# tan9zj/xnrs

Hardware: AMD Instinct MI355X
Metric: impressions/sec (encode+score) on MIND-shaped batches (higher is better)
Workload: dtype f32; 1 GPU; NRMS full user+news encode + 5-candidate dot scoring (BASELINE configs[2]; token shape of config/mind_small_NRMS.yml); batch_impressions_per_gpu=512, history=50, candidates=5, d_backbone=768, n_heads=16, emb_dim=256, parallelism=impressions sharded by user over 1 GPU(s), no data-path collective

## Files before the change

### include/xnrs_hip.h

```cpp
#ifndef XNRS_HIP_H
#define XNRS_HIP_H

#include <stddef.h>
#include <stdint.h>

#ifdef __cplusplus
extern "C" {
#endif

#define XNRS_ABI_VERSION 6

#define XNRS_OK 0
#define XNRS_EINVAL (-1)
#define XNRS_EHEADS (-2)
#define XNRS_EWORKSPACE (-3)
#define XNRS_EUNSUPPORTED (-4)

#define XNRS_ACT_NONE 0
#define XNRS_ACT_RELU 1
#define XNRS_ACT_TANH 2

#define XNRS_POOL_ADDITIVE 0
#define XNRS_POOL_MEAN 1

// ... 210 lines not shown

#define XNRS_PROFILE_STAGES 10
int32_t xnrs_profile_enable(uint32_t stage_mask);
int32_t xnrs_profile_read(double *ms, int64_t *launches, double *flops);

int32_t xnrs_qkv_launch_count(int32_t reset);
int32_t xnrs_qkv_one_launch_map(int64_t block, int64_t live_tiles, int64_t live_rows, int32_t kv_row_tiles,
                                int32_t kv_col_tiles, int64_t q_rows, int32_t q_tile_rows, int32_t q_col_tiles,
                                int32_t *section, int32_t *index);

int32_t xnrs_fc1_in_tail_count(int32_t reset);
int32_t xnrs_qkv_fc1_launch_map(int64_t block, int64_t live_tiles, int64_t live_rows, int64_t fc1_live_rows,
                                int32_t kv_row_tiles, int32_t kv_col_tiles, int64_t q_rows, int32_t q_tile_rows,
                                int32_t q_col_tiles, int64_t fc1_rows, int32_t fc1_tile_rows, int32_t fc1_col_tiles,
                                int32_t *section, int32_t *index);

int32_t xnrs_train_fold_enabled(void);

#define XNRS_STATUS_NONBINARY_MASK 1
#define XNRS_STATUS_ROW_RANGE 2
#define XNRS_STATUS_QUERY_RANGE 4
int32_t xnrs_set_status_word(int32_t *device_word);
const char *xnrs_status_string(int32_t word);

#define XNRS_GEMM_F32 0
#define XNRS_GEMM_BF16X3 1
#define XNRS_GEMM_BF16X2 2
int32_t xnrs_set_gemm_mode(int32_t mode);
int32_t xnrs_get_gemm_mode(void);

// ... 136 lines not shown
```

### xnrs_amd/csrc/api.hip

```cpp
#include <mutex>
#include <vector>

#include "host.h"

using namespace xnrs;

namespace xnrs {
uint32_t g_prof_mask = 0;
}
namespace {
std::vector<ProfRec> g_prof;
std::mutex g_prof_mu;
constexpr size_t PROF_MAX = 1 << 16;
}

bool xnrs::prof_begin(ProfRec* r, hipStream_t stream) {
  if (hipEventCreate(&r->beg) != hipSuccess || hipEventCreate(&r->end) != hipSuccess) return false;
  (void)hipEventRecord(r->beg, stream);
  return true;
}

void xnrs::prof_end(const ProfRec& r, hipStream_t stream) {
  (void)hipEventRecord(r.end, stream);
  std::lock_guard<std::mutex> lk(g_prof_mu);
// ... 79 lines not shown
  if (grid > 0x7fffffffLL) return XNRS_EINVAL;
  if (section && index) {
    const xnrs::QkvOneLaunchWork w =
        xnrs::qkv_one_launch_map(block, live_tiles, live_rows, kv_row_tiles, kv_col_tiles, q_rows, q_tile_rows, q_col_tiles);
    *section = w.section;
    *index = w.index;
  }
  return (int32_t)grid;
}

int32_t xnrs_fc1_in_tail_count(int32_t reset) {
  const int64_t n = xnrs::fc1_in_tail_read(reset != 0);
  return n > 0x7fffffffLL ? 0x7fffffff : (int32_t)n;
}

int32_t xnrs_qkv_fc1_launch_map(int64_t block, int64_t live_tiles, int64_t live_rows, int64_t fc1_live_rows, int32_t kv_row_tiles,
                                int32_t kv_col_tiles, int64_t q_rows, int32_t q_tile_rows, int32_t q_col_tiles, int64_t fc1_rows,
                                int32_t fc1_tile_rows, int32_t fc1_col_tiles, int32_t* section, int32_t* index) {
  if (kv_row_tiles < 0 || kv_col_tiles < 1 || q_rows < 0 || q_tile_rows < 1 || q_col_tiles < 1 || fc1_rows < 0 || fc1_tile_rows < 1 ||
      fc1_col_tiles < 1)
    return XNRS_EINVAL;
  const int64_t grid =
      xnrs::qkv_fc1_launch_grid(kv_row_tiles, kv_col_tiles, q_rows, q_tile_rows, q_col_tiles, fc1_rows, fc1_tile_rows, fc1_col_tiles);
  if (grid > 0x7fffffffLL) return XNRS_EINVAL;
  if (section && index) {
    const xnrs::QkvOneLaunchWork w = xnrs::qkv_fc1_launch_map(block, live_tiles, live_rows, fc1_live_rows, kv_row_tiles, kv_col_tiles, q_rows,
                                                              q_tile_rows, q_col_tiles, fc1_rows, fc1_tile_rows, fc1_col_tiles);
    *section = w.section;
    *index = w.index;
  }
// ... 42 lines not shown
```

### xnrs_amd/csrc/batch.hip

```cpp
#include <atomic>

#include "host.h"

namespace xnrs {

__device__ __forceinline__ uint64_t mix64(uint64_t seed, uint64_t a, uint64_t b) {
  uint64_t z = seed + 0x9E3779B97F4A7C15ull * (a * 0x100000001B3ull + b + 1);
  z = (z ^ (z >> 30)) * 0xBF58476D1CE4E5B9ull;
  z = (z ^ (z >> 27)) * 0x94D049BB133111EBull;
  return z ^ (z >> 31);
}

__global__ __launch_bounds__(256) void assemble_train_kernel(BatchArgs a) {
  const int64_t i = (int64_t)blockIdx.x * 256 + threadIdx.x;
  const int W = a.l_hist + 1 + a.n_neg;
  if (i >= a.B * W) return;
  const int64_t b = i / W;
  const int j = (int)(i - b * W);
  const int64_t s = a.sess[b];
  if (j < a.l_hist) {
    const int64_t lo = a.hist_off[s], hi = a.hist_off[s + 1];
    const int64_t n = (hi - lo < a.l_hist) ? (hi - lo) : a.l_hist;
    a.hist_out[b * a.l_hist + j] = (j < n) ? a.hist_val[hi - n + j] : a.pad_row;
  } else {
// ... 395 lines not shown
        w += __popcll(b);
        if (kept && sl < S) kv_src[e1 + sl] = (int32_t)(src0 + sl);
      }
      if (lane == 0) kv_block[j] = e1 / S;
    }
    __syncthreads();
  }
  bad = __syncthreads_or(bad);
  if (tid == 0) {
    counts[0] = s_carry[0];
    counts[1] = s_carry[1];
    counts[2] = bad ? 1 : 0;
  }
}

struct DenseLists {
  int32_t* live_loc;
  uint8_t* alive;
  int64_t* n_tiles;
  int32_t* tiles;
  int64_t cap;
  int BM;
};
__device__ void list_live_tiles(const uint8_t* __restrict__ alive, int64_t cn, int L, int BM, int32_t* __restrict__ tiles,
                                int64_t* __restrict__ n_out, int* s_wsum, int* s_carry);

template <bool DENSE>
__global__ __launch_bounds__(1024) void compact_rows64_kernel(const float* __restrict__ mask, const int32_t* __restrict__ ids,
                                                               int64_t n_news, int64_t chunk, int S, int64_t* __restrict__ row_off_all,
                                                               int32_t* __restrict__ live_all, int32_t* __restrict__ kvs_all,
                                                               int32_t* __restrict__ kvb_all, int64_t* __restrict__ counts_all,
                                                               DenseLists dl) {
  __shared__ unsigned long long s_bits[1024];
  __shared__ int64_t s_row[1024];
  __shared__ int s_ex[2][1024];
  __shared__ int s_wsum[2][16];
  __shared__ int s_carry[2];
  const int tid = threadIdx.x, wave = tid >> 6, lane = tid & 63;
  const int64_t news0 = (int64_t)blockIdx.x * chunk;
  const int cn = (int)(n_news - news0 < chunk ? n_news - news0 : chunk);
  int64_t* row_off = DENSE ? nullptr : row_off_all + (int64_t)blockIdx.x * (chunk + 1);
  int32_t* live_src = live_all ? live_all + (int64_t)blockIdx.x * chunk * S : nullptr;
  int32_t* kv_src = DENSE ? nullptr : kvs_all + (int64_t)blockIdx.x * chunk * S;
  int32_t* kv_block = DENSE ? nullptr : kvb_all + (int64_t)blockIdx.x * chunk;
  int64_t* counts = counts_all + 3 * (int64_t)blockIdx.x;
  int32_t* live_loc = DENSE ? dl.live_loc + (int64_t)blockIdx.x * chunk * S : nullptr;
  uint8_t* alive = DENSE ? dl.alive + news0 : nullptr;
  int bad = 0;
  if (tid < 2) s_carry[tid] = 0;
  if (!DENSE && tid == 0) row_off[0] = 0;
  for (int base = 0; base < cn; base += 1024) {
    const int nn = cn - base < 1024 ? cn - base : 1024;
    s_bits[tid] = 0ull;
    s_row[tid] = tid < nn ? (ids ? (int64_t)ids[news0 + base + tid] : news0 + base + tid) : 0;
    __syncthreads();
    const int n_el = nn * S;
    for (int i0 = tid; i0 < n_el; i0 += 4096) {
      float mv[4];
      int jj[4], sl[4];
#pragma unroll
      for (int u = 0; u < 4; ++u) {
        const int i = i0 + 1024 * u;
        jj[u] = (i < n_el ? i : 0) / S;
        sl[u] = (i < n_el ? i : 0) - jj[u] * S;
        mv[u] = i < n_el ? mask[s_row[jj[u]] * S + sl[u]] : 0.f;
// ... 13 lines not shown
      int x = v[which];
      for (int off = 1; off < 64; off <<= 1) {
        const int up = __shfl_up(x, off);
        if (lane >= off) x += up;
      }
      incl[which] = x;
      if (lane == 63) s_wsum[which][wave] = x;
    }
    __syncthreads();
    for (int which = 0; which < 2; ++which) {
      int before = s_carry[which];
      for (int w = 0; w < wave; ++w) before += s_wsum[which][w];
      s_ex[which][tid] = before + incl[which] - v[which];
    }
    if (tid < nn) {
      if constexpr (DENSE) {
        alive[base + tid] = bits != 0ull ? 1 : 0;
      } else {
        row_off[base + tid + 1] = s_ex[0][tid] + cnt;
        kv_block[base + tid] = s_ex[1][tid] / S;
      }
    }
    __syncthreads();
    if (tid == 1023) {
      s_carry[0] = s_ex[0][1023] + v[0];
      s_carry[1] = s_ex[1][1023] + v[1];
    }
#pragma unroll 4
    for (int i = tid; i < n_el; i += 1024) {
      const int jj = i / S, sl = i - jj * S;
      const unsigned long long b = s_bits[jj];
      if (b == 0ull) continue;
      const int32_t src = (int32_t)(s_row[jj] * S + sl);
      if constexpr (DENSE) {
        if ((b >> sl) & 1ull) {
          const int at = s_ex[0][jj] + __popcll(b & ((1ull << sl) - 1ull));
          live_loc[at] = (int32_t)((base + jj) * S + sl);
          if (live_src) live_src[at] = src;
        }
      } else {
        kv_src[s_ex[1][jj] + sl] = src;
        if ((b >> sl) & 1ull) live_src[s_ex[0][jj] + __popcll(b & ((1ull << sl) - 1ull))] = src;
      }
    }
    __syncthreads();
  }
  if constexpr (DENSE) {
    if (tid == 0) {
      counts[0] = s_carry[0];
      counts[1] = s_carry[1];
      s_carry[0] = 0;
    }
    __syncthreads();
    list_live_tiles(alive, cn, S, dl.BM, dl.tiles + (int64_t)blockIdx.x * dl.cap, dl.n_tiles + blockIdx.x, s_wsum[0], &s_carry[0]);
    return;
  }
  bad = __syncthreads_or(bad);
  if (tid == 0) {
    counts[0] = s_carry[0];
    counts[1] = s_carry[1];
    counts[2] = bad ? 1 : 0;
  }
}

__global__ __launch_bounds__(256) void row_counts_kernel(const float* __restrict__ mask, const int32_t* __restrict__ ids,
                                                          int64_t n_seq, int L, int32_t* __restrict__ cnt) {
  const int lane = threadIdx.x & 63;
  const int64_t seq = (int64_t)blockIdx.x * 4 + (threadIdx.x >> 6);
  if (seq >= n_seq) return;
  const float* mp = mask + (ids ? (int64_t)ids[seq] : seq) * L;
// ... 126 lines not shown
  return w;
}
void set_status_word(int32_t* w) {
  int dev = -1;
  (void)hipGetDevice(&dev);
  g_status_device.store(w ? dev : -1, std::memory_order_relaxed);
  g_status_word.store(w, std::memory_order_relaxed);
}

hipError_t launch_compact_rows(const float* mask, const int32_t* ids, int64_t n_news, int64_t chunk, int S, int64_t* row_off,
                               int32_t* live_src, int32_t* kv_src, int32_t* kv_block, int64_t* counts, hipStream_t stream) {
  if (n_news <= 0 || chunk <= 0) return hipSuccess;
  const int64_t passes = (n_news + chunk - 1) / chunk;
  if (passes > 0x7fffffffLL) return hipErrorInvalidValue;
  if (S <= 64)
    hipLaunchKernelGGL(compact_rows64_kernel<false>, dim3((unsigned)passes), dim3(1024), 0, stream, mask, ids, n_news, chunk, S,
                       row_off, live_src, kv_src, kv_block, counts, DenseLists{});
  else
    hipLaunchKernelGGL(compact_rows_kernel, dim3((unsigned)passes), dim3(1024), 0, stream, mask, ids, n_news, chunk, S, row_off,
                       live_src, kv_src, kv_block, counts);
  return hipGetLastError();
}

__global__ __launch_bounds__(1024) void live_tiles_kernel(const float* __restrict__ mask, const int32_t* __restrict__ ids,
                                                           int64_t n_seq, int64_t chunk, int L, int BM, int64_t cap,
                                                           uint8_t* __restrict__ alive_all, int64_t* __restrict__ n_tiles,
                                                           int32_t* __restrict__ tiles_all) {
  __shared__ int s_wsum[16];
  __shared__ int s_carry;
  const int tid = threadIdx.x;
  const int64_t seq0 = (int64_t)blockIdx.x * chunk;
  const int64_t cn = n_seq - seq0 < chunk ? n_seq - seq0 : chunk;
  uint8_t* alive = alive_all + seq0;
  int32_t* tiles = tiles_all + (int64_t)blockIdx.x * cap;
  for (int64_t j = tid; j < cn; j += 1024) {
    const float* mp = mask + (ids ? (int64_t)ids[seq0 + j] : seq0 + j) * L;
    int any = 0;
// ... 35 lines not shown
  }
  if (tid == 0) *n_out = *s_carry;
}

hipError_t launch_live_tiles(const float* mask, const int32_t* ids, int64_t n_seq, int64_t chunk, int L, int BM, uint8_t* alive,
                             int64_t* n_tiles, int32_t* tiles, hipStream_t stream) {
  if (n_seq <= 0 || chunk <= 0 || L <= 0 || BM <= 0) return hipSuccess;
  const int64_t passes = (n_seq + chunk - 1) / chunk;
  const int64_t cap = live_tiles_cap(chunk, L, BM);
  if (passes > 0x7fffffffLL || cap > 0x7fffffffLL) return hipErrorInvalidValue;
  hipLaunchKernelGGL(live_tiles_kernel, dim3((unsigned)passes), dim3(1024), 0, stream, mask, ids, n_seq, chunk, L, BM, cap, alive,
                     n_tiles, tiles);
  return hipGetLastError();
}

hipError_t launch_dense_row_lists(const float* mask, const int32_t* ids, int64_t n_seq, int64_t chunk, int L, int BM,
                                  int32_t* live_loc, int32_t* live_src, int64_t* counts, uint8_t* alive, int64_t* n_tiles,
                                  int32_t* tiles, hipStream_t stream) {
  if (n_seq <= 0 || chunk <= 0 || L <= 0 || BM <= 0) return hipSuccess;
  const int64_t passes = (n_seq + chunk - 1) / chunk;
  const int64_t cap = live_tiles_cap(chunk, L, BM);
  if (L > 64 || passes > 0x7fffffffLL || cap > 0x7fffffffLL || chunk * L > 0x7fffffffLL) return hipErrorInvalidValue;
  hipLaunchKernelGGL(compact_rows64_kernel<true>, dim3((unsigned)passes), dim3(1024), 0, stream, mask, ids, n_seq, chunk, L,
                     nullptr, ids ? live_src : nullptr, nullptr, nullptr, counts, DenseLists{live_loc, alive, n_tiles, tiles, cap, BM});
  return hipGetLastError();
}

}

using namespace xnrs;

extern "C" {

size_t xnrs_row_lists_workspace_bytes(int64_t n_seq) { return n_seq > 0 ? align_up((size_t)n_seq * sizeof(int32_t)) : 0; }

int32_t xnrs_build_row_lists(const float* m, const int32_t* ids, int64_t n_seq, int32_t L, int32_t* live_rows,
                             int32_t* live_src_rows, int32_t* kv_rows, int32_t* kv_src_rows, int64_t* counts, void* ws,
                             size_t ws_bytes, void* stream) {
  if (n_seq < 0 || L <= 0 || !m || !live_rows || !kv_rows || !counts) return XNRS_EINVAL;
// ... 92 lines not shown
```

### xnrs_amd/csrc/encoder_fwd.hip

```cpp
#include <vector>

#include "host.h"

using namespace xnrs;

namespace xnrs {

Plan make_plan(int64_t n_seq, int L, int D, int A, int E, bool att, bool additive, bool head, bool pooled, int64_t chunk,
               bool train, int n_heads, bool widen) {
  Plan p{};
  if (train) chunk = n_seq > 0 ? n_seq : 1;
  if (chunk <= 0) chunk = 65536 / L;
  if (chunk > n_seq) chunk = n_seq;
  if (chunk < 1) chunk = 1;
  p.chunk = chunk;
  const size_t rows = (size_t)chunk * L;
  Carver c;
  p.off_qkv = c.take_if(att, rows * 3 * (size_t)D * F32);
  p.off_o = c.take_if(att, rows * (size_t)D * F32);
  p.off_y = c.take_if(att && pooled, rows * (size_t)D * F32);
  p.off_t = c.take_if(pooled && additive, rows * (size_t)A * F32);
  p.off_p = c.take_if(pooled && head, (size_t)n_seq * D * F32);
  p.off_h = c.take_if(pooled && head, (size_t)n_seq * E * F32);
  p.off_stats = c.take_if(train && att, (size_t)chunk * n_heads * L * 2 * F32);
// ... 210 lines not shown
    if (is_additive(r) && (!r.pool || !r.pool->w1 || !r.pool->w2 || r.pool->hidden <= 0)) return XNRS_EINVAL;
    if (r.pool_kind == XNRS_POOL_MEAN && !r.m) return XNRS_EINVAL;
    if (r.L > 512) return XNRS_EUNSUPPORTED;
    if (r.head && (!r.head->w0 || !r.head->w2 || r.head->out_features <= 0 || r.head->activation < 0 || r.head->activation > 2))
      return XNRS_EINVAL;
  }
  return (r.ids && !r.m && r.pooled && r.pool_kind == XNRS_POOL_MEAN) ? XNRS_EINVAL : XNRS_OK;
}

struct Route {
  bool fused, afused;
  bool qkv_given, live, kvl, lr_qkv, tail, lt_qkv, direct, a16;
  bool fold;
  bool lr_fc1, lt_fc1, rowdot;
  bool skip_dead, read_counts;
};

bool news_fused_route(const SeqEncode& r, const Plan& p, int A, bool fold, NewsFusedArgs* f) {
  const xnrs_mha_params* att = r.att;
  const int L = r.L, D = r.D;
  if (!(att && is_additive(r) && !r.train && !r.a_out && att->dropout_p == 0.f && gemm_mode() == 0 && knobs().news_fused &&
        news_fused_plan(L, D, att->n_heads, A, nullptr) && (D / att->n_heads) * att->n_heads == D &&
        (knobs().news_fused == 2 || (L >= 26 && r.n_seq >= 192))))
    return false;
  f->x = r.x; f->ids = r.ids; f->mask = r.m;
  f->wq = att->wq; f->bq = att->bq; f->wk = att->wk; f->bk = att->bk; f->wv = att->wv; f->bv = att->bv;
  f->wo = att->wo; f->bo = att->bo;
  f->w1 = r.pool->w1; f->b1 = r.pool->b1; f->w2 = r.pool->w2; f->b2 = r.pool->b2;
  f->img = at(r.ws, p.off_nf);
  f->p = pooled_dst(fold, at(r.ws, p.fold.po), r.head, at(r.ws, p.off_p), r.y);
// ... 49 lines not shown
                  device_counts_ok(xal, D, A, r.att, additive ? r.pool : nullptr);
  MhaCoreArgs probe{};
  if (lt && knobs().mha_skip_masked) {
    probe = mha_core_args(at(r.ws, p.off_qkv) + D, 3 * (int64_t)D, r.att, at(r.ws, p.off_o), p.chunk, L, D);
    probe.q = at(r.ws, p.off_qkv); probe.mask = r.m; probe.skip_dead = 1;
  }
  rt.lt_qkv = probe.skip_dead && mha_core_skips_dead(probe);
  rt.lt_fc1 = lt && additive && rt.rowdot;
  const bool lr = lt && knobs().gemm_live_rows && p.off_lr_cnt != 0 && L <= 64 && n_rows <= 0x7fffffffLL &&
                  n_rows >= knobs().gemm_live_rows_min_rows;
  rt.lr_qkv = lr && rt.lt_qkv && !rt.direct;
  rt.lr_fc1 = lr && rt.lt_fc1;
  rt.tail = rt.lr_qkv && rt.lr_fc1 && rt.fold && r.pooled && !r.ids && !r.x16 && knobs().gemm_fc1_in_tail && !prof_on(3);
  rt.read_counts = (rt.lt_qkv && prof_on(0)) || (rt.lt_fc1 && prof_on(3));
  rt.skip_dead = rt.live || (r.pooled && r.m && knobs().mha_skip_masked);
  return rt;
}

struct Call {
  const SeqEncode& r;
  hipStream_t stream;
  const Plan p;
  const Route rt;
  NewsFusedArgs nf; AdditiveFusedArgs af;
  const int L = r.L, D = r.D, A = hidden_of(r);
  const xnrs_mha_params* att = r.att;
  const xnrs_row_lists rl = r.rl ? *r.rl : xnrs_row_lists{};
  const int32_t *lvx = rt.live ? (r.ids ? rl.live_src_rows : rl.live_rows) : nullptr, *kvx = rt.kvl ? (r.ids ? rl.kv_src_rows : rl.kv_rows) : nullptr;
  const int64_t* cnt = rl.counts_dev;
  const int64_t n_live = cnt ? r.n_seq * L : rl.n_live, n_kv = cnt ? r.n_seq * L : rl.n_kv;
// ... 167 lines not shown
int32_t project(const Call& c, const Pass& pass, DeferredFc1* prev) {
  if (c.rt.qkv_given) return XNRS_OK;
  if (c.rt.live) return project_train_lists(c, pass);
  if (c.rt.lr_qkv) return project_live_rows(c, pass, prev);
  GemmArgs g = qkv_projection(pass.cx, {pass.xids, c.L}, c.att, 0, c.qkv, 3 * (int64_t)c.D, pass.rows, c.D, c.pqkv);
  if (c.rt.lt_qkv) over_live_tiles(&g, pass.ltn, pass.ltl);
  ProfScope ps(0, 2.0 * (c.rt.lt_qkv ? pass.lt_rows : (double)pass.rows) * 3.0 * c.D * c.D, c.stream);
  return hip_rc(c.rt.direct ? launch_gemm_a16(g, c.r.x16, c.stream) : launch_gemm_f32(g, c.stream));
}

int32_t attend(const Call& c, const Pass& pass) {
  MhaCoreArgs ma = mha_core_args(c.qkv + c.D, 3 * (int64_t)c.D, c.att, c.o, pass.nc, c.L, c.D);
  ma.q = c.qkv; ma.mask = pass.cm; ma.mask_gather_ids = pass.cids; ma.dropout_p = c.att->dropout_p;
  ma.seed = c.att->seed + (uint64_t)pass.c0 * (uint64_t)c.att->n_heads * 0x9E3779B97F4A7C15ull;
  ma.seed_dev = c.att->seed_dev; ma.stats = c.stats; ma.skip_dead = c.rt.skip_dead ? 1 : 0;
  if (c.rt.lt_qkv && !mha_core_skips_dead(ma)) return XNRS_EUNSUPPORTED;
  ProfScope ps(1, 4.0 * pass.rows * (double)c.L * c.D, c.stream);
  return hip_rc(launch_mha_core(ma, c.stream));
}

int32_t out_project_train_lists(const Call& c, const Pass& pass, float* dst) {
  const int D = c.D;
  ProfScope ps(2, 2.0 * (double)prof_count(2, c.cnt, 0, c.n_live, c.stream) * (double)D * D, c.stream);
  XNRS_TRY(hipMemsetAsync(dst, 0, (size_t)pass.rows * D * sizeof(float), c.stream));
  if (c.n_live <= 0) return XNRS_OK;
  GemmArgs og = gemm_linear(c.o, {}, D, c.att->wo, c.att->bo, dst, D, 0, D, D, XNRS_ACT_NONE, c.po);
  over_row_list(&og, c.rl.live_rows, nullptr, c.n_live, c.cnt, 0.4f);
  return hip_rc(launch_gemm_f32(og, c.stream));
}
int32_t out_project(const Call& c, Pass* pass) {
  float* dst = c.rt.fold ? c.o : (c.r.pooled ? c.yb : c.r.y + pass->c0 * (int64_t)c.L * c.D);
  pass->seq = dst; pass->seq_ids = nullptr;
  if (c.rt.fold) return XNRS_OK;
// ... 459 lines not shown
```

### xnrs_amd/csrc/gemm_f32.hip

```cpp
#include <atomic>
#include <cstdlib>
#include <type_traits>

#include "kernels.h"

namespace xnrs {

constexpr int KALIGN = 32;

__device__ __attribute__((aligned(16))) float g_zero_line[4] = {0.f, 0.f, 0.f, 0.f};

typedef unsigned u32x4 __attribute__((ext_vector_type(4)));
constexpr unsigned BUF_OOB = 0x40000000u;

template <int TM, int TN, bool A_COL, bool B_KN, bool VEC, int PIPE, int BK, bool BUF = false, int MINW = 2, bool GATH = false,
          int KG = 2, bool RDOT = false, bool MDEV = false, bool LIVE = false>
__global__ __launch_bounds__(256, MINW) void gemm_f32_kernel(const GemmArgs a, int m_tiles, int n_tiles_seg, int gn) {
#define XNRS_GEMM_BID blockIdx.x
#define XNRS_GEMM_NWG gridDim.x
#define XNRS_GEMM_LDS_TILES(A, B)                            \
  __shared__ __attribute__((aligned(16))) float A[NBUF][A_SZ]; \
  __shared__ __attribute__((aligned(16))) float B[NBUF][B_SZ];
#include "gemm_f32_body.h"
#undef XNRS_GEMM_BID
// ... 323 lines not shown
  k.mha_lds = (int)num("XNRS_MHA_LDS", -1);
  k.mha_headwave = num("XNRS_MHA_HEADWAVE", 1) != 0;
  k.mha_pair = num("XNRS_MHA_PAIR", 1) != 0;
  k.mha_bwd_fused = num("XNRS_MHA_BWD_FUSED", 1) != 0;
  k.gemm_dw = (int)num("XNRS_GEMM_DW", 2);
  k.gemm_dw_tile = (int)num("XNRS_GEMM_DW_TILE", 256);
  k.fold_out = (int)num("XNRS_FOLD_OUT", 1);
  k.fc1_rowdot = num("XNRS_FC1_ROWDOT", 1) != 0;
  k.fold_train = (int)num("XNRS_FOLD_TRAIN", 1);
  k.news_fused = (int)num("XNRS_NEWS_FUSED", 1);
  k.news_fused_npw = (int)num("XNRS_NEWS_FUSED_NPW", 0);
  k.fast_tanh = num("XNRS_FAST_TANH", 1) != 0;
  k.additive_fused = (int)num("XNRS_ADDITIVE_FUSED", 1);
  k.af_fbuf = num("XNRS_AF_FBUF", 1) == 2 ? 2 : 1;
  k.mha_skip_masked = num("XNRS_MHA_SKIP_MASKED", 1) != 0;
  {
    k.gemm_qkv_one_launch = num("XNRS_GEMM_QKV_ONE_LAUNCH", 1) != 0;
  }
  k.gemm_fc1_in_tail = num("XNRS_GEMM_FC1_IN_TAIL", 1) != 0;
  k.gemm_live_tiles = num("XNRS_GEMM_LIVE_TILES", 1) != 0;
  k.gemm_live_tiles_min_rows = num("XNRS_GEMM_LIVE_TILES_MIN_ROWS", 16384);
  k.gemm_live_rows = num("XNRS_GEMM_LIVE_ROWS", 1) != 0;
  k.gemm_live_rows_min_rows = num("XNRS_GEMM_LIVE_ROWS_MIN_ROWS", 16384);
  k.bwd_side_stream = num("XNRS_BWD_SIDE_STREAM", 1) != 0;
  k.bwd_side_min_rows = num("XNRS_BWD_SIDE_MIN_ROWS", 0);
  k.gru_layout = num("XNRS_GRU_LAYOUT", 0) == 1 ? 1 : 0;
  k.gemm_a16 = num("XNRS_GEMM_A16", 1) != 0;
  const long long m = num("XNRS_GEMM_MODE", 0);
  k.gemm_mode_init = (m >= 0 && m <= 2) ? (int)m : 0;
  return k;
// ... 157 lines not shown
```

### xnrs_amd/csrc/kernels.h

```cpp
#pragma once
#include <hip/hip_runtime.h>
#include <stdint.h>

namespace xnrs {

typedef float f32x4 __attribute__((ext_vector_type(4)));
typedef float f32x16 __attribute__((ext_vector_type(16)));
inline bool aligned16(const void* p) { return (reinterpret_cast<uintptr_t>(p) & 15) == 0; }

struct Knobs {
  int gemm_pipe = 6;
  int gemm_bk = 32;
  int gemm_buf = 1;
  long long gemm_group = -1;
  int gemm_tile = -1;
  long long split_min_tiles = 512;
  bool fc1_rowdot = true;
  int fold_train = 1;
  int fold_out = 1;
  int gemm_dw = 2;
  int gemm_dw_tile = 256;
  int mha_lds = -1;
  bool mha_pair = true;
  int mha_headwave = 1;
// ... 1 lines not shown
  int news_fused = 1;
  int news_fused_npw = 0;
  int gemm_mode_init = 0;
  bool fast_tanh = true;
  int additive_fused = 1;
  int af_fbuf = 1;
  bool bwd_side_stream = true;
  long long bwd_side_min_rows = 0;
  bool gemm_live_tiles = true;
  long long gemm_live_tiles_min_rows = 16384;
  bool gemm_live_rows = true;
  long long gemm_live_rows_min_rows = 16384;
  bool gemm_qkv_one_launch = true;
  bool gemm_fc1_in_tail = true;
  bool mha_skip_masked = true;
  bool gemm_a16 = true;
  int gru_layout = 0;
};
const Knobs& knobs();
void reload_knobs();

__device__ __forceinline__ int64_t load_dev_scalar(const int64_t* p) { return *p; }

struct GemmArgs {
  const float* A;
  int32_t a_col;
  const int32_t* gather_ids;
  int32_t gather_S;
  int32_t c_scatter;
  const int32_t* c_scatter_ids;
// ... 110 lines not shown
  const float* mask;
  const int32_t* mask_gather_ids;
  float* out;
  int64_t ldo;
  int64_t n_seq;
  int32_t S, n_heads, d_k;
  int32_t scaled;
  float dropout_p;
  uint64_t seed;
  const uint64_t* seed_dev;
  float* stats;
  const int64_t* q_off;
  int64_t ldq;
  const int32_t* kv_block;
  int32_t skip_dead;
};
hipError_t launch_mha_core(const MhaCoreArgs& a, hipStream_t stream);
bool mha_core_skips_dead(const MhaCoreArgs& a);

struct MhaBwdArgs {
  const float* q;
  const float* k;
  const float* v;
  int64_t ld;
  const float* mask;
  const int32_t* mask_gather_ids;
  const float* o;
  int64_t ldo;
  const float* d_o;
  int64_t lddo;
  const float* stats;
  float* delta;
  float* dq;
// ... 332 lines not shown
```

### xnrs_amd/csrc/mha_core.hip

```cpp
#include <cstdlib>

#include "kernels.h"

namespace xnrs {

template <int KT, bool VEC>
__global__ __launch_bounds__(256) void mha_core_kernel(MhaCoreArgs a, int QT, int64_t n_units) {
  const int lane = threadIdx.x & 63;
  const int64_t unit = (int64_t)blockIdx.x * 4 + (threadIdx.x >> 6);
  if (unit >= n_units) return;
  const int qt = (int)(unit % QT);
  const int64_t uh = unit / QT;
  const int hd = (int)(uh % a.n_heads);
  const int64_t seq = uh / a.n_heads;

  const int c = lane & 15, g = lane >> 4;
  const int S = a.S, dk = a.d_k;
  const int64_t row0 = seq * S;
  const int hoff = hd * dk;
  const int query = qt * 16 + c;
  const bool qvalid = query < S;

  f32x4 acc[KT];
#pragma unroll
// ... 423 lines not shown
  const float* vbase = a.v + kvbase;
  const int rem = TAIL ? S - KTM * 16 : 0;

  const int64_t q0 = a.q_off ? a.q_off[seq] : (int64_t)seq * S;
  const int nq = a.q_off ? (int)(a.q_off[seq + 1] - q0) : S;
  const int QT = (nq + 15) >> 4;
  if (nq == 0) return;
  const int c = lane & 15, g = lane >> 4;
  const int query = qt * 16 + c;
  const bool qvalid = query < nq;
  float mq = 1.f;
  if (a.mask && !a.q_off && qvalid) {
    const int64_t mrow = a.mask_gather_ids ? (int64_t)a.mask_gather_ids[seq] * S : (int64_t)seq * S;
    mq = a.mask[mrow + query];
  }
  if (a.skip_dead && a.mask && !a.q_off) {
    if (!__syncthreads_or(qvalid && mq != 0.f)) {
      if (qvalid) {
        float* orow = a.out + (q0 + query) * a.ldo + hd * dk;
#pragma unroll
        for (int dt = 0; dt < NFB; ++dt) {
          const int dv0 = dt * 16 + 4 * g;
          if (dv0 < dk) *reinterpret_cast<f32x4*>(orow + dv0) = f32x4{0.f, 0.f, 0.f, 0.f};
        }
        if (a.stats && g == 0) {
          float* sp = a.stats + (((int64_t)seq * a.n_heads + hd) * (int64_t)S + query) * 2;
          sp[0] = -1e9f;
          sp[1] = (float)S;
        }
      }
      return;
    }
  }
  const bool tile_dead = a.skip_dead && a.mask && !a.q_off && !__any(qvalid && mq != 0.f);
  const float* qrow = a.q_off ? a.q + (q0 + (qvalid ? query : 0)) * a.ldq + hd * dk
                              : a.q + hbase + (int64_t)(qvalid ? query : 0) * ld;
  f32x4 qf[NFB];
#pragma unroll
// ... 45 lines not shown
        }
      } else if (TAIL) {
#pragma unroll
        for (int r = 0; r < 4; ++r) Vt[r * NCH + vch] = vv[r];
      }
    }
  }
  __syncthreads();
  if (qt >= QT) return;
  if (tile_dead) {
    if (qvalid) {
      float* orow0 = a.out + (q0 + query) * a.ldo + hd * dk;
#pragma unroll
      for (int dt = 0; dt < NFB; ++dt) {
        const int dv0 = dt * 16 + 4 * g;
        if (dv0 < dk) *reinterpret_cast<f32x4*>(orow0 + dv0) = f32x4{0.f, 0.f, 0.f, 0.f};
      }
      if (a.stats && g == 0) {
        float* sp = a.stats + (((int64_t)seq * a.n_heads + hd) * (int64_t)S + query) * 2;
        sp[0] = -1e9f;
        sp[1] = (float)S;
      }
    }
    return;
  }

  f32x4 acc[KTM];
#pragma unroll
  for (int kt = 0; kt < KTM; ++kt) acc[kt] = f32x4{0.f, 0.f, 0.f, 0.f};
#pragma unroll
  for (int fb = 0; fb < NFB; ++fb) {
// ... 104 lines not shown
  if constexpr (TAIL) {
#pragma unroll
    for (int t = 0; t < 4; ++t) {
      if (t < rem) {
#pragma unroll
        for (int dt = 0; dt < NFB; ++dt) {
          const f32x4 vr = Vt[t * NCH + dt * 4 + g];
#pragma unroll
          for (int r = 0; r < 4; ++r) o[dt][r] = fmaf(st[t], vr[r], o[dt][r]);
        }
      }
    }
  }
  const int hoff = hd * dk;
  float* orow = a.out + (q0 + query) * a.ldo + hoff;
#pragma unroll
  for (int dt = 0; dt < NFB; ++dt) {
    const int dv0 = dt * 16 + 4 * g;
    if (qvalid && dv0 < dk) *reinterpret_cast<f32x4*>(orow + dv0) = o[dt];
  }
}

template <int KTM, int NFB, bool TAIL>
static hipError_t launch_pair_nfb(const MhaCoreArgs& a, hipStream_t stream) {
  const int64_t n_pairs = a.n_seq * a.n_heads;
  if (n_pairs > 0x7fffffffLL) return hipErrorInvalidValue;
  if (a.dropout_p > 0.f)
    hipLaunchKernelGGL((mha_core_pair_kernel<KTM, NFB, TAIL, true>), dim3((unsigned)n_pairs), dim3(256), 0, stream, a);
  else
    hipLaunchKernelGGL((mha_core_pair_kernel<KTM, NFB, TAIL, false>), dim3((unsigned)n_pairs), dim3(256), 0, stream, a);
  return hipGetLastError();
}

template <int KTM, bool TAIL>
// ... 42 lines not shown
  p.KT = (a.S + 15) / 16;
  p.fast = p.vec && a.S <= 64 && a.d_k <= 64 && ((int64_t)a.S * a.ld < (1ll << 31)) && knobs().mha_headwave;
  p.use_lds = a.q_off ? true : (knobs().mha_lds >= 0 ? knobs().mha_lds != 0 : (p.KT >= 3));
  const int rem = a.S & 15;
  p.tail = a.S > 16 && rem >= 1 && rem <= 4;
  p.KTM = p.tail ? a.S >> 4 : p.KT;
  p.pair = p.fast && p.use_lds && knobs().mha_pair && (int64_t)a.n_seq * a.S < (1ll << 31) &&
           (p.tail ? (p.KTM == 2 || p.KTM == 3) : (p.KTM == 3 || p.KTM == 4));
  return p;
}

bool mha_core_skips_dead(const MhaCoreArgs& a) {
  return a.skip_dead && a.mask && !a.q_off && a.S <= 128 && mha_pick(a).pair;
}

hipError_t launch_mha_core(const MhaCoreArgs& a, hipStream_t stream) {
  if (a.n_seq <= 0 || a.S <= 0) return hipSuccess;
  if (a.S > 128) return hipErrorInvalidValue;
  const MhaPick pk = mha_pick(a);
  const bool vec = pk.vec, fast = pk.fast, use_lds = pk.use_lds;
  const int KT = pk.KT;
  if (a.q_off && (!fast || a.stats || a.dropout_p > 0.f || a.ldq % 4 != 0)) return hipErrorInvalidValue;
  if (pk.pair) {
    const bool tail = pk.tail;
    const int KTM = pk.KTM;
    if (tail && KTM == 2) return launch_pair<2, true>(a, stream);
    if (tail && KTM == 3) return launch_pair<3, true>(a, stream);
    if (!tail && KTM == 3) return launch_pair<3, false>(a, stream);
    if (!tail && KTM == 4) return launch_pair<4, false>(a, stream);
  }
  if (fast && use_lds) {
    switch (KT) {
      case 1: return launch_lds_kt<1, 1>(a, stream);
      case 2: return launch_lds_kt<2, 2>(a, stream);
      case 3: return launch_lds_kt<3, 4>(a, stream);
      default: return launch_lds_kt<4, 4>(a, stream);
    }
// ... 23 lines not shown
```

Before: 21500 impressions/s.

## Skip attention output stores for masked rows and parallelize dense row lists

Adds an o_live_only mode to the pair MHA kernel. When a downstream fused path only reads live rows, it skips writing outputs for masked queries and dead sequences, which cuts global stores. It also replaces the single-block-per-pass dense row-list compaction with a new kernel that splits each pass into 64-row slices across many blocks. Each slice recomputes its prefix counts by rescanning earlier rows, so work is spread out at the cost of redundant mask reads. Masked output rows are now left uninitialized, which is only safe if every consumer reads live rows only.

```diff
diff --git a/include/xnrs_hip.h b/include/xnrs_hip.h
--- a/include/xnrs_hip.h
+++ b/include/xnrs_hip.h
@@ -248,6 +248,8 @@
                                 int32_t kv_row_tiles, int32_t kv_col_tiles, int64_t q_rows, int32_t q_tile_rows,
                                 int32_t q_col_tiles, int64_t fc1_rows, int32_t fc1_tile_rows, int32_t fc1_col_tiles,
                                 int32_t *section, int32_t *index);
+
+int32_t xnrs_mha_live_o_count(int32_t reset);
 
 int32_t xnrs_train_fold_enabled(void);
 
diff --git a/xnrs_amd/csrc/api.hip b/xnrs_amd/csrc/api.hip
--- a/xnrs_amd/csrc/api.hip
+++ b/xnrs_amd/csrc/api.hip
@@ -117,6 +117,11 @@
   return n > 0x7fffffffLL ? 0x7fffffff : (int32_t)n;
 }
 
+int32_t xnrs_mha_live_o_count(int32_t reset) {
+  const int64_t n = xnrs::mha_live_o_read(reset != 0);
+  return n > 0x7fffffffLL ? 0x7fffffff : (int32_t)n;
+}
+
 int32_t xnrs_qkv_fc1_launch_map(int64_t block, int64_t live_tiles, int64_t live_rows, int64_t fc1_live_rows, int32_t kv_row_tiles,
                                 int32_t kv_col_tiles, int64_t q_rows, int32_t q_tile_rows, int32_t q_col_tiles, int64_t fc1_rows,
                                 int32_t fc1_tile_rows, int32_t fc1_col_tiles, int32_t* section, int32_t* index) {
diff --git a/xnrs_amd/csrc/batch.hip b/xnrs_amd/csrc/batch.hip
--- a/xnrs_amd/csrc/batch.hip
+++ b/xnrs_amd/csrc/batch.hip
@@ -1,4 +1,5 @@
 #include <atomic>
+#include <type_traits>
 
 #include "host.h"
 
@@ -433,23 +434,10 @@
   }
 }
 
-struct DenseLists {
-  int32_t* live_loc;
-  uint8_t* alive;
-  int64_t* n_tiles;
-  int32_t* tiles;
-  int64_t cap;
-  int BM;
-};
-__device__ void list_live_tiles(const uint8_t* __restrict__ alive, int64_t cn, int L, int BM, int32_t* __restrict__ tiles,
-                                int64_t* __restrict__ n_out, int* s_wsum, int* s_carry);
-
-template <bool DENSE>
 __global__ __launch_bounds__(1024) void compact_rows64_kernel(const float* __restrict__ mask, const int32_t* __restrict__ ids,
                                                                int64_t n_news, int64_t chunk, int S, int64_t* __restrict__ row_off_all,
                                                                int32_t* __restrict__ live_all, int32_t* __restrict__ kvs_all,
-                                                               int32_t* __restrict__ kvb_all, int64_t* __restrict__ counts_all,
-                                                               DenseLists dl) {
+                                                               int32_t* __restrict__ kvb_all, int64_t* __restrict__ counts_all) {
   __shared__ unsigned long long s_bits[1024];
   __shared__ int64_t s_row[1024];
   __shared__ int s_ex[2][1024];
@@ -458,16 +446,14 @@
   const int tid = threadIdx.x, wave = tid >> 6, lane = tid & 63;
   const int64_t news0 = (int64_t)blockIdx.x * chunk;
   const int cn = (int)(n_news - news0 < chunk ? n_news - news0 : chunk);
-  int64_t* row_off = DENSE ? nullptr : row_off_all + (int64_t)blockIdx.x * (chunk + 1);
-  int32_t* live_src = live_all ? live_all + (int64_t)blockIdx.x * chunk * S : nullptr;
-  int32_t* kv_src = DENSE ? nullptr : kvs_all + (int64_t)blockIdx.x * chunk * S;
-  int32_t* kv_block = DENSE ? nullptr : kvb_all + (int64_t)blockIdx.x * chunk;
+  int64_t* row_off = row_off_all + (int64_t)blockIdx.x * (chunk + 1);
+  int32_t* live_src = live_all + (int64_t)blockIdx.x * chunk * S;
+  int32_t* kv_src = kvs_all + (int64_t)blockIdx.x * chunk * S;
+  int32_t* kv_block = kvb_all + (int64_t)blockIdx.x * chunk;
   int64_t* counts = counts_all + 3 * (int64_t)blockIdx.x;
-  int32_t* live_loc = DENSE ? dl.live_loc + (int64_t)blockIdx.x * chunk * S : nullptr;
-  uint8_t* alive = DENSE ? dl.alive + news0 : nullptr;
   int bad = 0;
   if (tid < 2) s_carry[tid] = 0;
-  if (!DENSE && tid == 0) row_off[0] = 0;
+  if (tid == 0) row_off[0] = 0;
   for (int base = 0; base < cn; base += 1024) {
     const int nn = cn - base < 1024 ? cn - base : 1024;
     s_bits[tid] = 0ull;
@@ -511,12 +497,8 @@
       s_ex[which][tid] = before + incl[which] - v[which];
     }
     if (tid < nn) {
-      if constexpr (DENSE) {
-        alive[base + tid] = bits != 0ull ? 1 : 0;
-      } else {
-        row_off[base + tid + 1] = s_ex[0][tid] + cnt;
-        kv_block[base + tid] = s_ex[1][tid] / S;
-      }
+      row_off[base + tid + 1] = s_ex[0][tid] + cnt;
+      kv_block[base + tid] = s_ex[1][tid] / S;
     }
     __syncthreads();
     if (tid == 1023) {
@@ -529,28 +511,10 @@
       const unsigned long long b = s_bits[jj];
       if (b == 0ull) continue;
       const int32_t src = (int32_t)(s_row[jj] * S + sl);
-      if constexpr (DENSE) {
-        if ((b >> sl) & 1ull) {
-          const int at = s_ex[0][jj] + __popcll(b & ((1ull << sl) - 1ull));
-          live_loc[at] = (int32_t)((base + jj) * S + sl);
-          if (live_src) live_src[at] = src;
-        }
-      } else {
-        kv_src[s_ex[1][jj] + sl] = src;
-        if ((b >> sl) & 1ull) live_src[s_ex[0][jj] + __popcll(b & ((1ull << sl) - 1ull))] = src;
-      }
-    }
-    __syncthreads();
-  }
-  if constexpr (DENSE) {
-    if (tid == 0) {
-      counts[0] = s_carry[0];
-      counts[1] = s_carry[1];
-      s_carry[0] = 0;
-    }
-    __syncthreads();
-    list_live_tiles(alive, cn, S, dl.BM, dl.tiles + (int64_t)blockIdx.x * dl.cap, dl.n_tiles + blockIdx.x, s_wsum[0], &s_carry[0]);
-    return;
+      kv_src[s_ex[1][jj] + sl] = src;
+      if ((b >> sl) & 1ull) live_src[s_ex[0][jj] + __popcll(b & ((1ull << sl) - 1ull))] = src;
+    }
+    __syncthreads();
   }
   bad = __syncthreads_or(bad);
   if (tid == 0) {
@@ -707,13 +671,16 @@
   const int64_t passes = (n_news + chunk - 1) / chunk;
   if (passes > 0x7fffffffLL) return hipErrorInvalidValue;
   if (S <= 64)
-    hipLaunchKernelGGL(compact_rows64_kernel<false>, dim3((unsigned)passes), dim3(1024), 0, stream, mask, ids, n_news, chunk, S,
-                       row_off, live_src, kv_src, kv_block, counts, DenseLists{});
+    hipLaunchKernelGGL(compact_rows64_kernel, dim3((unsigned)passes), dim3(1024), 0, stream, mask, ids, n_news, chunk, S, row_off,
+                       live_src, kv_src, kv_block, counts);
   else
     hipLaunchKernelGGL(compact_rows_kernel, dim3((unsigned)passes), dim3(1024), 0, stream, mask, ids, n_news, chunk, S, row_off,
                        live_src, kv_src, kv_block, counts);
   return hipGetLastError();
 }
+
+__device__ void list_live_tiles(const uint8_t* __restrict__ alive, int64_t cn, int L, int BM, int32_t* __restrict__ tiles,
+                                int64_t* __restrict__ n_out, int* s_wsum, int* s_carry);
 
 __global__ __launch_bounds__(1024) void live_tiles_kernel(const float* __restrict__ mask, const int32_t* __restrict__ ids,
                                                            int64_t n_seq, int64_t chunk, int L, int BM, int64_t cap,
@@ -779,15 +746,127 @@
   return hipGetLastError();
 }
 
+constexpr int DL_SLICE = 64;
+constexpr int DL_ROWS = 16;
+__global__ __launch_bounds__(1024, 8) void dense_row_lists_kernel(const float* __restrict__ mask, const int32_t* __restrict__ ids,
+                                                                int64_t n_news, int64_t chunk, int S, int nsl,
+                                                                int32_t* __restrict__ live_loc_all, int32_t* __restrict__ live_src_all,
+                                                                int64_t* __restrict__ counts_all, uint8_t* __restrict__ alive_all,
+                                                                int64_t* __restrict__ n_tiles, int32_t* __restrict__ tiles_all,
+                                                                int64_t cap, int BM) {
+  __shared__ unsigned long long s_bits[DL_SLICE];
+  __shared__ int32_t s_row[DL_SLICE];
+  __shared__ int s_ex[DL_SLICE];
+  __shared__ int s_part[2][16];
+  __shared__ int s_wsum[16];
+  __shared__ int s_carry;
+  const int tid = threadIdx.x, lane = tid & 63;
+  const int wave = __builtin_amdgcn_readfirstlane(tid >> 6);
+  const int64_t pass = blockIdx.x / nsl;
+  const int slice = blockIdx.x % nsl;
+  const int64_t news0 = pass * chunk;
+  const int cn = (int)(n_news - news0 < chunk ? n_news - news0 : chunk);
+  const int j0 = slice * DL_SLICE;
+  if (j0 >= cn) return;
+  const int j1 = j0 + DL_SLICE < cn ? j0 + DL_SLICE : cn;
+  const bool last = j1 == cn;
+  if (tid < DL_SLICE) {
+    s_bits[tid] = 0ull;
+    s_row[tid] = 0;
+  }
+  __syncthreads();
+  int before = 0, kept = 0;
+  const int lc = lane < S ? lane : S - 1;
+  auto sweep = [&](auto gathered) {
+    for (int jb = wave; jb < j1; jb += 16 * DL_ROWS) {
+      int32_t row[DL_ROWS];
+      float mv[DL_ROWS];
+#pragma unroll
+      for (int u = 0; u < DL_ROWS; ++u) {
+        const int jc = jb + 16 * u < j1 ? jb + 16 * u : j1 - 1;
+        if constexpr (decltype(gathered)::value)
+          row[u] = ids[news0 + jc];
+        else
+          row[u] = (int32_t)(news0 + jc);
+      }
+#pragma unroll
+      for (int u = 0; u < DL_ROWS; ++u) mv[u] = mask[(int64_t)row[u] * S + lc];
+#pragma unroll
+      for (int u = 0; u < DL_ROWS; ++u) {
+        const int j = jb + 16 * u;
+        const unsigned long long b = __ballot(lane < S && mv[u] != 0.f);
+        if (j >= j1) continue;
+        if (j < j0) {
+          before += __popcll(b);
+          kept += b != 0ull ? 1 : 0;
+        } else if (lane == 0) {
+          s_bits[j - j0] = b;
+          s_row[j - j0] = row[u];
+        }
+        if (last && lane == 0) alive_all[news0 + j] = b != 0ull ? 1 : 0;
+      }
+    }
+  };
+  if (ids)
+    sweep(std::true_type{});
+  else
+    sweep(std::false_type{});
+  if (lane == 0) {
+    s_part[0][wave] = before;
+    s_part[1][wave] = kept;
+  }
+  __syncthreads();
+  if (wave == 0) {
+    const unsigned long long bits = s_bits[lane];
+    const int cnt = __popcll(bits);
+    int x = cnt;
+    for (int off = 1; off < 64; off <<= 1) {
+      const int up = __shfl_up(x, off);
+      if (lane >= off) x += up;
+    }
+    int base = 0, kbase = 0;
+    for (int w = 0; w < 16; ++w) {
+      base += s_part[0][w];
+      kbase += s_part[1][w];
+    }
+    s_ex[lane] = base + x - cnt;
+    const int kown = __popcll(__ballot(bits != 0ull));
+    if (last && lane == 63) {
+      int64_t* counts = counts_all + 3 * pass;
+      counts[0] = base + x;
+      counts[1] = (int64_t)(kbase + kown) * S;
+    }
+  }
+  __syncthreads();
+  int32_t* live_loc = live_loc_all + pass * chunk * S;
+  int32_t* live_src = live_src_all ? live_src_all + pass * chunk * S : nullptr;
+  const int n_el = (j1 - j0) * S;
+  for (int i = tid; i < n_el; i += 1024) {
+    const int jj = i / S, sl = i - jj * S;
+    const unsigned long long b = s_bits[jj];
+    if (!((b >> sl) & 1ull)) continue;
+    const int at = s_ex[jj] + __popcll(b & ((1ull << sl) - 1ull));
+    live_loc[at] = (int32_t)((j0 + jj) * S + sl);
+    if (live_src) live_src[at] = (int32_t)((int64_t)s_row[jj] * S + sl);
+  }
+  if (!last) return;
+  if (tid == 0) s_carry = 0;
+  __syncthreads();
+  list_live_tiles(alive_all + news0, cn, S, BM, tiles_all + pass * cap, n_tiles + pass, s_wsum, &s_carry);
+}
+
 hipError_t launch_dense_row_lists(const float* mask, const int32_t* ids, int64_t n_seq, int64_t chunk, int L, int BM,
                                   int32_t* live_loc, int32_t* live_src, int64_t* counts, uint8_t* alive, int64_t* n_tiles,
                                   int32_t* tiles, hipStream_t stream) {
   if (n_seq <= 0 || chunk <= 0 || L <= 0 || BM <= 0) return hipSuccess;
   const int64_t passes = (n_seq + chunk - 1) / chunk;
   const int64_t cap = live_tiles_cap(chunk, L, BM);
-  if (L > 64 || passes > 0x7fffffffLL || cap > 0x7fffffffLL || chunk * L > 0x7fffffffLL) return hipErrorInvalidValue;
-  hipLaunchKernelGGL(compact_rows64_kernel<true>, dim3((unsigned)passes), dim3(1024), 0, stream, mask, ids, n_seq, chunk, L,
-                     nullptr, ids ? live_src : nullptr, nullptr, nullptr, counts, DenseLists{live_loc, alive, n_tiles, tiles, cap, BM});
+  if (L > 64 || passes > 0x7fffffffLL || cap > 0x7fffffffLL || chunk * L > 0x7fffffffLL || n_seq > 0x7fffffffLL) return hipErrorInvalidValue;
+  const int64_t per_pass = chunk < n_seq ? chunk : n_seq;
+  const int64_t nsl = (per_pass + DL_SLICE - 1) / DL_SLICE;
+  if (passes * nsl > 0x7fffffffLL) return hipErrorInvalidValue;
+  hipLaunchKernelGGL(dense_row_lists_kernel, dim3((unsigned)(passes * nsl)), dim3(1024), 0, stream, mask, ids, n_seq, chunk, L,
+                     (int)nsl, live_loc, ids ? live_src : nullptr, counts, alive, n_tiles, tiles, cap, BM);
   return hipGetLastError();
 }
 
diff --git a/xnrs_amd/csrc/encoder_fwd.hip b/xnrs_amd/csrc/encoder_fwd.hip
--- a/xnrs_amd/csrc/encoder_fwd.hip
+++ b/xnrs_amd/csrc/encoder_fwd.hip
@@ -248,6 +248,7 @@
   bool fold;
   bool lr_fc1, lt_fc1, rowdot;
   bool skip_dead, read_counts;
+  bool o_live;
 };
 
 bool news_fused_route(const SeqEncode& r, const Plan& p, int A, bool fold, NewsFusedArgs* f) {
@@ -327,6 +328,7 @@
   rt.tail = rt.lr_qkv && rt.lr_fc1 && rt.fold && r.pooled && !r.ids && !r.x16 && knobs().gemm_fc1_in_tail && !prof_on(3);
   rt.read_counts = (rt.lt_qkv && prof_on(0)) || (rt.lt_fc1 && prof_on(3));
   rt.skip_dead = rt.live || (r.pooled && r.m && knobs().mha_skip_masked);
+  rt.o_live = rt.lr_fc1 && rt.lt_qkv && rt.fold && r.pooled && !r.train && rt.skip_dead && r.att->dropout_p == 0.f && knobs().mha_live_o;
   return rt;
 }
 
@@ -524,9 +526,12 @@
   ma.q = c.qkv; ma.mask = pass.cm; ma.mask_gather_ids = pass.cids; ma.dropout_p = c.att->dropout_p;
   ma.seed = c.att->seed + (uint64_t)pass.c0 * (uint64_t)c.att->n_heads * 0x9E3779B97F4A7C15ull;
   ma.seed_dev = c.att->seed_dev; ma.stats = c.stats; ma.skip_dead = c.rt.skip_dead ? 1 : 0;
+  ma.o_live_only = c.rt.o_live ? 1 : 0;
   if (c.rt.lt_qkv && !mha_core_skips_dead(ma)) return XNRS_EUNSUPPORTED;
   ProfScope ps(1, 4.0 * pass.rows * (double)c.L * c.D, c.stream);
-  return hip_rc(launch_mha_core(ma, c.stream));
+  XNRS_TRY(launch_mha_core(ma, c.stream));
+  if (c.rt.o_live) mha_live_o_add(1);
+  return XNRS_OK;
 }
 
 int32_t out_project_train_lists(const Call& c, const Pass& pass, float* dst) {
diff --git a/xnrs_amd/csrc/gemm_f32.hip b/xnrs_amd/csrc/gemm_f32.hip
--- a/xnrs_amd/csrc/gemm_f32.hip
+++ b/xnrs_amd/csrc/gemm_f32.hip
@@ -361,6 +361,7 @@
   k.additive_fused = (int)num("XNRS_ADDITIVE_FUSED", 1);
   k.af_fbuf = num("XNRS_AF_FBUF", 1) == 2 ? 2 : 1;
   k.mha_skip_masked = num("XNRS_MHA_SKIP_MASKED", 1) != 0;
+  k.mha_live_o = num("XNRS_MHA_LIVE_O", 1) != 0;
   {
     k.gemm_qkv_one_launch = num("XNRS_GEMM_QKV_ONE_LAUNCH", 1) != 0;
   }
diff --git a/xnrs_amd/csrc/kernels.h b/xnrs_amd/csrc/kernels.h
--- a/xnrs_amd/csrc/kernels.h
+++ b/xnrs_amd/csrc/kernels.h
@@ -39,6 +39,7 @@
   bool gemm_qkv_one_launch = true;
   bool gemm_fc1_in_tail = true;
   bool mha_skip_masked = true;
+  bool mha_live_o = true;
   bool gemm_a16 = true;
   int gru_layout = 0;
 };
@@ -179,9 +180,12 @@
   int64_t ldq;
   const int32_t* kv_block;
   int32_t skip_dead;
+  int32_t o_live_only;
 };
 hipError_t launch_mha_core(const MhaCoreArgs& a, hipStream_t stream);
 bool mha_core_skips_dead(const MhaCoreArgs& a);
+void mha_live_o_add(int n);
+int64_t mha_live_o_read(bool reset);
 
 struct MhaBwdArgs {
   const float* q;
diff --git a/xnrs_amd/csrc/mha_core.hip b/xnrs_amd/csrc/mha_core.hip
--- a/xnrs_amd/csrc/mha_core.hip
+++ b/xnrs_amd/csrc/mha_core.hip
@@ -1,3 +1,4 @@
+#include <atomic>
 #include <cstdlib>
 
 #include "kernels.h"
@@ -461,6 +462,7 @@
     const int64_t mrow = a.mask_gather_ids ? (int64_t)a.mask_gather_ids[seq] * S : (int64_t)seq * S;
     mq = a.mask[mrow + query];
   }
+  const bool o_live = !DROP && a.o_live_only && a.skip_dead && a.mask && !a.q_off;
   if (a.skip_dead && a.mask && !a.q_off) {
     if (!__syncthreads_or(qvalid && mq != 0.f)) {
       if (qvalid) {
@@ -468,7 +470,7 @@
 #pragma unroll
         for (int dt = 0; dt < NFB; ++dt) {
           const int dv0 = dt * 16 + 4 * g;
-          if (dv0 < dk) *reinterpret_cast<f32x4*>(orow + dv0) = f32x4{0.f, 0.f, 0.f, 0.f};
+          if (!o_live && dv0 < dk) *reinterpret_cast<f32x4*>(orow + dv0) = f32x4{0.f, 0.f, 0.f, 0.f};
         }
         if (a.stats && g == 0) {
           float* sp = a.stats + (((int64_t)seq * a.n_heads + hd) * (int64_t)S + query) * 2;
@@ -544,7 +546,7 @@
 #pragma unroll
       for (int dt = 0; dt < NFB; ++dt) {
         const int dv0 = dt * 16 + 4 * g;
-        if (dv0 < dk) *reinterpret_cast<f32x4*>(orow0 + dv0) = f32x4{0.f, 0.f, 0.f, 0.f};
+        if (!o_live && dv0 < dk) *reinterpret_cast<f32x4*>(orow0 + dv0) = f32x4{0.f, 0.f, 0.f, 0.f};
       }
       if (a.stats && g == 0) {
         float* sp = a.stats + (((int64_t)seq * a.n_heads + hd) * (int64_t)S + query) * 2;
@@ -679,10 +681,11 @@
   }
   const int hoff = hd * dk;
   float* orow = a.out + (q0 + query) * a.ldo + hoff;
+  const bool stored = qvalid && !(o_live && mq == 0.f);
 #pragma unroll
   for (int dt = 0; dt < NFB; ++dt) {
     const int dv0 = dt * 16 + 4 * g;
-    if (qvalid && dv0 < dk) *reinterpret_cast<f32x4*>(orow + dv0) = o[dt];
+    if (stored && dv0 < dk) *reinterpret_cast<f32x4*>(orow + dv0) = o[dt];
   }
 }
 
@@ -755,6 +758,12 @@
   return a.skip_dead && a.mask && !a.q_off && a.S <= 128 && mha_pick(a).pair;
 }
 
+static std::atomic<int64_t> g_mha_live_o{0};
+void mha_live_o_add(int n) { g_mha_live_o.fetch_add(n, std::memory_order_relaxed); }
+int64_t mha_live_o_read(bool reset) {
+  return reset ? g_mha_live_o.exchange(0, std::memory_order_relaxed) : g_mha_live_o.load(std::memory_order_relaxed);
+}
+
 hipError_t launch_mha_core(const MhaCoreArgs& a, hipStream_t stream) {
   if (a.n_seq <= 0 || a.S <= 0) return hipSuccess;
   if (a.S > 128) return hipErrorInvalidValue;
@@ -762,6 +771,7 @@
   const bool vec = pk.vec, fast = pk.fast, use_lds = pk.use_lds;
   const int KT = pk.KT;
   if (a.q_off && (!fast || a.stats || a.dropout_p > 0.f || a.ldq % 4 != 0)) return hipErrorInvalidValue;
+  if (a.o_live_only && (a.stats || a.dropout_p > 0.f || !mha_core_skips_dead(a))) return hipErrorInvalidValue;
   if (pk.pair) {
     const bool tail = pk.tail;
     const int KTM = pk.KTM;
```

Result: faster. 21940 impressions/s, median of 6 (+2.0%).
